# JuanLuisGonzalez/FAL_net

Hardware: AMD Instinct MI355X
Metric: stereo-pairs/sec Stage-1 step @256x512 N=49 (higher is better)
Workload: dtype bf16; 1 GPU; Stage-1 training step (BASELINE configs[1]), batch 8/GPU, 256x512, N=49, seeded weights, seeded VGG19; global_batch=8, parallelism=dp1, launch=eager launches, recorded sequences issued by falnet_replay (C)

## Files before the change

### fal_net_amd/_lib.py

```python
import ctypes as C
import os
import threading

import torch

F32, BF16, F16 = 0, 1, 2
ACT_NONE, ACT_ELU, ACT_RELU = 0, 1, 2
OUT_NHWC, OUT_PLANAR_F32 = 0, 1
CPAD = 32

DETERMINISTIC = os.environ.get("FALNET_DETERMINISTIC") == "1"

def ab(name, default):
    if os.environ.get("FALNET_AB") != "1":
        return default
    return os.environ.get(name, default)


_LIB_PATH = os.environ.get("FALNET_LIB") or os.path.join(os.path.dirname(os.path.abspath(__file__)), "libfalnet_hip.so")


class Src(C.Structure):
    _fields_ = [("ptr", C.c_void_p), ("C", C.c_int32), ("H", C.c_int32), ("W", C.c_int32),
                ("sb", C.c_int64), ("sy", C.c_int64), ("sx", C.c_int64)]


class Conv(C.Structure):
    _fields_ = [("src", Src * 2), ("nsrc", C.c_int32), ("IH", C.c_int32), ("IW", C.c_int32),
                ("weight", C.c_void_p), ("cin_total", C.c_int32), ("ntaps", C.c_int32),
                ("tap_dy", C.c_int32 * 9), ("tap_dx", C.c_int32 * 9), ("tap_w", C.c_int32 * 9),
                ("w_taps", C.c_int32), ("w_rows", C.c_int32), ("isy", C.c_int32), ("isx", C.c_int32),
                ("B", C.c_int32), ("TH", C.c_int32), ("TW", C.c_int32),
                ("osy", C.c_int32), ("osx", C.c_int32), ("ooy", C.c_int32), ("oox", C.c_int32),
                ("out", C.c_void_p), ("OH", C.c_int32), ("OW", C.c_int32), ("Cout", C.c_int32),
                ("out_cstride", C.c_int32), ("out_layout", C.c_int32), ("bias", C.c_void_p),
                ("addend", C.c_void_p), ("act", C.c_int32), ("actout", C.c_void_p),
                ("actout_kind", C.c_int32), ("dtype", C.c_int32), ("ksplit", C.c_int32), ("splitk_ws", C.c_void_p),
                ("splitk_ws_bytes", C.c_int64), ("variant", C.c_int32), ("pool_out", C.c_void_p),
                ("pool_mode", C.c_int32), ("pool_actout_kind", C.c_int32), ("pool_actout", C.c_void_p), ("weight_up2", C.c_void_p),
                ("scratch", C.c_void_p), ("scratch_bytes", C.c_int64), ("pool_code", C.c_void_p)]


class Wgrad(C.Structure):
    _fields_ = [("src", Src * 2), ("nsrc", C.c_int32), ("IH", C.c_int32), ("IW", C.c_int32),
                ("gout", C.c_void_p), ("gC", C.c_int32), ("ntaps", C.c_int32),
                ("tap_dy", C.c_int32 * 9), ("tap_dx", C.c_int32 * 9), ("isy", C.c_int32), ("isx", C.c_int32),
                ("B", C.c_int32), ("TH", C.c_int32), ("TW", C.c_int32), ("cin_total", C.c_int32),
                ("nsplit", C.c_int32), ("partial", C.c_void_p), ("dtype", C.c_int32), ("variant", C.c_int32), ("bias_grad", C.c_void_p),
                ("cout", C.c_int32), ("up2", C.c_int32)]


class ReduceDesc(C.Structure):
    _fields_ = [("partial", C.c_void_p), ("grad", C.c_void_p), ("nsplit", C.c_int32), ("ntaps", C.c_int32),
                ("w_rows", C.c_int32), ("cin_total", C.c_int32), ("cout", C.c_int32), ("cin", C.c_int32),
                ("c0_real", C.c_int32), ("c0_pad", C.c_int32), ("groups", C.c_int32), ("block_begin", C.c_int32)]


class PackDesc(C.Structure):
    _fields_ = [("w", C.c_void_p), ("wf", C.c_void_p), ("wd", C.c_void_p), ("cout", C.c_int32), ("cin", C.c_int32),
                ("taps", C.c_int32), ("c0_real", C.c_int32), ("c0_pad", C.c_int32), ("cin_pad", C.c_int32),
                ("cout_pad", C.c_int32), ("block_begin", C.c_int32), ("no_update", C.c_int32), ("reserved", C.c_int32)]


# ... 407 lines not shown
```

### fal_net_amd/csrc/conv.hip

```cpp
#include <limits.h>
#include <stdlib.h>
#include <type_traits>
#include "common.h"
#include "conv_epilogue.h"

#define CONV_THREADS 256
#define CONV_BM 128
#define ROWB 64
#define ROWP 80

template <typename T> struct KC;
template <> struct KC<float> { static constexpr int value = 16; };
template <> struct KC<bf16_t> { static constexpr int value = 32; };
template <> struct KC<f16_t> { static constexpr int value = 32; };

template <typename T, int MT, int NT, typename RowOff, typename PoolOff = NoPool>
__device__ __forceinline__ void epilogue_nhwc(const falnet_conv_t& p, f32x16 (&acc)[MT][NT], float* stage, int nbase, int lane,
                                              RowOff rowoff, PoolOff pooloff = PoolOff()) {
    constexpr bool POOL = !std::is_same<PoolOff, NoPool>::value;
    constexpr int PITCHF = NT * 32 + 4;
    constexpr int CS = NT * 4;
    constexpr int RPP = 64 / CS;
    constexpr int PASSES = 32 / RPP;
    const int r = lane & 31, h = lane >> 5;
// ... 1466 lines not shown
        }
        flip = fwd ? 0 : (bwd ? 1 : -1);
    }
    dense3x3 = dense3x3 && flip >= 0;
    const int esz = p.dtype == FALNET_F32 ? 4 : 2;
    bool c128 = true;
    for (int s = 0; s < p.nsrc; ++s) c128 = c128 && (p.src[s].C % (128 / esz) == 0);
    int variant = p.variant;
    int forced_bn = 0;
    if (variant == 11 || variant == 12) {
        forced_bn = variant == 11 ? 32 : 64;
        if (p.w_rows % forced_bn != 0 || p.pool_out) {
            falnet_set_error("conv2d: variant %d (gather, %d channels per workgroup) not applicable to this launch", variant, forced_bn);
            return -2;
        }
        variant = 1;
    }
    if (p.pool_code && !(variant == 23 && p.dtype != FALNET_F32 && p.pool_out && p.pool_mode == 0 && !planar && p.OH % 2 == 0 && p.OW % 2 == 0 &&
                         p.Cout % 32 == 0 && p.out_cstride % 32 == 0)) {
        falnet_set_error("conv2d: pool_code (argmax codes of the fused max pool) needs variant 23, a 16-bit type, pool_out with pool_mode 0, an NHWC "
                         "launch with even OH / OW and whole 32-channel groups (variant %d, dtype %d, pool_mode %d)", p.variant, p.dtype, p.pool_mode);
        return -2;
    }
    if (g_disable_patch) variant = 1;
    switch (variant) {
        case 0: case 1: case 2: case 3: case 4: case 5: case 6: case 7: case 8: case 9: case 10:
        case 13: case 15: case 16: case 17: case 18: case 19: case 20: case 21: case 22: case 23: case 24: case 25: case 26: case 27: case 29:
            break;
        default:
            falnet_set_error("conv2d: unknown variant %d", variant);
            return -1;
    }
    if (variant == 19) {
        if (!falnet_conv_deep_applicable(p)) {
            falnet_set_error("conv2d: variant 19 needs a 16-bit nine-tap stride-1/2 launch on maps of at most 128 positions (128 %% (TH TW) == 0), dense NHWC output, "
                             "w_rows %% 64 == 0, ksplit = cin_total / 32 or / 64 (a multiple of 4), scratch for the partial tiles and the split-K workspace");
            return -2;
        }
        c.flip = 0;
        c.swap = 0;
        c.family = ConvFamily::Deep;
        c.bn = 64; c.kcb = p.ksplit * 32 == p.cin_total ? 1 : 2; c.tps = 9; c.adb = 1; c.th = 0; c.nwaves = falnet_conv_deep_mtiles(p);
        return 0;
    }
    if (variant == 15) {
        if (!falnet_conv_s2f_dma_applicable(p)) {
// ... 234 lines not shown
static int ws_symbol(char* buf, int len, const char* t, const falnet_conv_t& p, const ConvChoice& c) {
    const int m16 = (int)(falnet_mfma16_enabled() && p.dtype != FALNET_F32);
    if (c.adb) return snprintf(buf, len, "_Z18conv3x3_ws2_kernelI%sLi%dELi%dELb%dELb%dEEv13falnet_conv_tiii", t, c.bn, c.kcb, m16, (int)(c.kcb == 2 && ws2_whole_lines(p)));
    return snprintf(buf, len, "_Z17conv3x3_ws_kernelI%sLi%dELi%dELb%dEEv13falnet_conv_tiii", t, c.bn, c.kcb, m16);
}

struct ConvFamilyRow {
    ConvFamily family;
    int (*symbol)(char* buf, int len, const char* t, const falnet_conv_t& p, const ConvChoice& c);
    int (*launch)(const falnet_conv_t& p, const ConvChoice& c, hipStream_t st);
};
#define SYMBOL(...) [](char* buf, int len, const char* t, const falnet_conv_t& p, const ConvChoice& c) { return snprintf(buf, len, __VA_ARGS__); }
#define LAUNCH(...) [](const falnet_conv_t& p, const ConvChoice& c, hipStream_t st) { return __VA_ARGS__; }
static const ConvFamilyRow conv_families[] = {
    {ConvFamily::Gather, SYMBOL("_Z17conv_igemm_kernelI%sLi%dELb%dEEv13falnet_conv_t", t, c.bn, c.swap), launch_gather},
    {ConvFamily::Patch, SYMBOL("_Z20conv3x3_patch_kernelI%sLi%dELi%dELi%dELb%dELi%dELi%dEEv13falnet_conv_tiii", t, c.bn, c.kcb, c.tps, c.adb, c.th, c.nwaves), launch_patch},
    {ConvFamily::WeightStationary, ws_symbol, launch_ws},
    {ConvFamily::Dma, SYMBOL("_Z18conv3x3_dma_kernelI%sLi%dELi%dEEv13falnet_conv_tiiii", t, c.th, c.nwaves), LAUNCH(falnet_conv_dma_launch(p, c.flip, st, c.th, c.max_wgs, c.count))},
    {ConvFamily::S2fDma, SYMBOL("_Z22conv3x3_s2f_dma_kernelI%sLi%dEEv13falnet_conv_tiii", t, c.bn), LAUNCH(falnet_conv_s2f_dma_launch(p, st, c.max_wgs, c.count))},
    {ConvFamily::Up2Dma, SYMBOL("_Z22conv3x3_up2_dma_kernelI%sEv13falnet_conv_tiiiii", t), LAUNCH(falnet_conv_up2_dma_launch(p, st, c.max_wgs, c.count))},
    {ConvFamily::Deep, SYMBOL("_Z19conv3x3_deep_kernelI%sLi%dELi%dEEv13falnet_conv_t18falnet_deep_geom_t", t, c.kcb, c.nwaves), LAUNCH(falnet_conv_deep_launch(p, st, c.count))},
    {ConvFamily::Dma2, SYMBOL("_Z19conv3x3_dma2_kernelI%sLb%dELi%dEEv13falnet_conv_tiiiii", t, p.pool_out ? 1 : 0, c.nwaves), LAUNCH(falnet_conv_dma2_launch(p, c.flip, st, c.th, c.max_wgs, c.count))},
    {ConvFamily::Dma16, [](char* buf, int len, const char* t, const falnet_conv_t& p, const ConvChoice& c) {
         if (p.pool_out && p.pool_code) return snprintf(buf, len, "_Z20conv3x3_dma16_kernelI9PoolCodesI%sELb1ELi16ELi8ELb0EEv13falnet_conv_tiiii", t);
         return snprintf(buf, len, "_Z20conv3x3_dma16_kernelI%sLb%dELi%dELi%dELb%dEEv13falnet_conv_tiiii", t, p.pool_out ? 1 : 0, c.th, c.nwaves, p.out_layout == FALNET_OUT_PLANAR_F32 ? 1 : 0);
     },
     LAUNCH(falnet_conv_dma16_launch(p, c.flip, st, c.th, c.max_wgs, c.count))},
    {ConvFamily::Up2d, SYMBOL("_Z25conv2x2_up2d_dma16_kernelI%sEv13falnet_conv_tiii", t), LAUNCH(falnet_conv_up2d_launch(p, st, c.max_wgs, c.count))},
    {ConvFamily::Wave32, SYMBOL("_Z21conv3x3_wave32_kernelI%sEv13falnet_conv_tiiii", t), LAUNCH(falnet_conv_wave32_launch(p, c.flip, st, c.count))},
    {ConvFamily::Wave64p, SYMBOL("_Z22conv3x3_wave64p_kernelI%sEv13falnet_conv_tiiii", t), LAUNCH(falnet_conv_wave64p_launch(p, c.flip, st, c.count))},
};
#undef SYMBOL
#undef LAUNCH

static const ConvFamilyRow* conv_family_row(ConvFamily f) {
    for (const ConvFamilyRow& r : conv_families)
        if (r.family == f) return &r;
    falnet_set_error("conv2d: kernel family %d has no table row", (int)f);
    return nullptr;
}

extern "C" int falnet_conv2d_kernel_name(const falnet_conv_t* pp, char* buf, int len) {
    FALNET_CHECK_ARG(pp && buf && len > 0, "conv2d_kernel_name: bad argument");
    ConvChoice c;
    if (int r = choose_conv_kernel(*pp, c)) return r;
    const ConvFamilyRow* row = conv_family_row(c.family);
// ... 155 lines not shown
```

### fal_net_amd/csrc/conv_dma.hip

```cpp
#include <stdlib.h>
#include "conv_epilogue.h"

#ifndef FALNET_DMA_ROW_REUSE
#define FALNET_DMA_ROW_REUSE 1
#endif
#ifndef FALNET_DMA_EPI_AHEAD
#define FALNET_DMA_EPI_AHEAD -1
#endif
#ifndef FALNET_DMA16_EPI_AHEAD
#define FALNET_DMA16_EPI_AHEAD 0
#endif

#define CD_ZERO_BYTES 32768
__device__ uint4 g_cd_zero[CD_ZERO_BYTES / 16] = {};

typedef __attribute__((address_space(3))) void* cd_lptr_t;

__device__ __forceinline__ void cd_glds16(const void* gsrc, unsigned lds_dst) {
    unsigned keep;
    asm volatile("s_mov_b32 %0, m0\n\ts_mov_b32 m0, %2\n\ts_nop 0\n\tglobal_load_lds_dwordx4 %1, off\n\ts_mov_b32 m0, %0"
                 : "=&s"(keep)
                 : "v"(gsrc), "s"(lds_dst)
                 : "memory");
}
// ... 535 lines not shown
    FALNET_COUNT_ONLY(count, gx * ny);
    static const int skew_pct = [] { const char* e = falnet_ab_env("FALNET_DMA2_SKEW"); return e ? atoi(e) : 0; }();
    int cin = 0;
    for (int s = 0; s < p.nsrc; ++s) cin += p.src[s].C;
    const int skew = (th == 16 && gx * ny > 256) ? (int)((int64_t)skew_pct * (cin / 16) * 5200 / 100 / 64) : 0;
#define DMA2_K(T, PL, NW) hipLaunchKernelGGL(HIP_KERNEL_NAME(conv3x3_dma2_kernel<T, PL, NW>), grid, dim3(NW * 64), 0, st, p, tiles_x, tiles_y, flip, ntiles, skew)
#define DMA2_L(T)                                              \
    do {                                                       \
        if (th == 32) {                                        \
            if (p.pool_out) DMA2_K(T, true, 8);                \
            else DMA2_K(T, false, 8);                          \
        } else {                                               \
            if (p.pool_out) DMA2_K(T, true, 4);                \
            else DMA2_K(T, false, 4);                          \
        }                                                      \
    } while (0)
    FALNET_DISPATCH_16(p.dtype, DMA2_L);
#undef DMA2_L
#undef DMA2_K
    FALNET_RETURN_LAUNCH();
}

template <typename T> struct PoolCodes {};
template <typename TT> struct Dma16Operand { typedef TT type; static constexpr bool codes = false; };
template <typename T> struct Dma16Operand<PoolCodes<T>> { typedef T type; static constexpr bool codes = true; };
template <typename TT, bool POOL, int TH, int NWAVES, bool PLANAR>
__global__ __launch_bounds__(NWAVES * 64, NWAVES == 8 ? 2 : 1) void conv3x3_dma16_kernel(const falnet_conv_t p, int tiles_x, int tiles_y, int flip, int ntiles) {
    typedef typename Dma16Operand<TT>::type T;
    constexpr bool CODES = Dma16Operand<TT>::codes;
    constexpr int MT = TH / NWAVES, BN = 64, NT = BN / 32;
    static_assert(sizeof(T) == 2 && (MT == 1 || MT == 2) && (MT == 2 || !POOL), "16-bit operands; one or two rows per wave; the fused pool needs row pairs");
    constexpr int KCV = 32;
    constexpr int NPIX = (TH + 2) * CD_PW;
    constexpr int A_PIECES = (NPIX + 15) / 16, B_PIECES = 9 * BN / 16, NPIECES = A_PIECES + B_PIECES;
    constexpr int A_BYTES = A_PIECES * 1024, BUF = NPIECES * 1024;
    constexpr int ROWB = CD_PW * 64;
    __shared__ __attribute__((aligned(1024))) char lds[2 * BUF];
    __shared__ __attribute__((aligned(16))) float lds_bias[BN];
    const int tid = threadIdx.x, lane = tid & 63;
    const int wave = __builtin_amdgcn_readfirstlane(tid >> 6);
    const unsigned lds_base = (unsigned)(unsigned long)(cd_lptr_t)lds;
    const int r = lane & 31, h = lane >> 5;
    const int lp = lane & 15, lg = lane >> 4;
    const int n0 = blockIdx.y * BN;
    const char* const zero_page = reinterpret_cast<const char*>(g_cd_zero);
    stage_bias_lds(p, n0, BN, lds_bias);

    const int nsrc = p.nsrc, IH = p.IH, IW = p.IW;
    const int C0 = p.src[0].C, C1 = nsrc > 1 ? p.src[1].C : 0;
    const int nchunks = (C0 + C1) / KCV;
    int my_tiles = 0;
    for (int t = blockIdx.x; t < ntiles; t += gridDim.x) ++my_tiles;
// ... 33 lines not shown
        t.tx += step_.tx;
        if (t.tx >= tiles_x) { t.tx -= tiles_x; ++t.ty; }
        t.ty += step_.ty;
        if (t.ty >= tiles_y) { t.ty -= tiles_y; ++t.b; }
        t.b += step_.b;
    };
    int pr_[KP], pc_[KP], a_lc[2][KP];
#pragma unroll
    for (int k = 0; k < KP; ++k) {
        const int pix = 16 * (wave + NWAVES * k) + l4;
        const int pr = pix / CD_PW, pc = pix - pr * CD_PW;
        pr_[k] = pix < NPIX ? pr : -(1 << 20);
        pc_[k] = pc;
#pragma unroll
        for (int s2 = 0; s2 < 2; ++s2) {
            const falnet_src_t& S = s2 == 0 ? p.src[0] : p.src[(nsrc > 1) ? 1 : 0];
            const int hs = S.H != IH ? 1 : 0, ws = S.W != IW ? 1 : 0;
            a_lc[s2][k] = ((pr - 1) >> hs) * (int)S.sy + ((pc - 1) >> ws) * (int)S.sx + (segpos ^ (((pc >> 2) & 1) << 1)) * 8;
        }
    }
    int a_off[KP];
    unsigned a_ok = 0;
    const T* a_base = sptr[0];
    auto tile_offsets = [&](const TPos& t, int s2) {
        const falnet_src_t& S = s2 == 0 ? p.src[0] : p.src[1];
        const int hs = S.H != IH ? 1 : 0, ws = S.W != IW ? 1 : 0;
        const int ty0 = t.ty * TH, tx0 = t.tx * 32;
        a_base = sptr[s2] + ((int64_t)t.b * S.sb + (int64_t)((ty0 >> hs) * (int)S.sy + (tx0 >> ws) * (int)S.sx));
        a_ok = 0;
#pragma unroll
        for (int k = 0; k < KP; ++k) {
            const int vy = ty0 - 1 + pr_[k], vx = tx0 - 1 + pc_[k];
            a_ok |= (vy >= 0 && vy < IH && vx >= 0 && vx < IW) ? 1u << k : 0u;
            a_off[k] = a_lc[s2][k];
        }
    };
    struct Cur { int tile, c, s, c0, kofs; TPos t; };
    auto advance = [&](Cur& q) {
        if (++q.c == nchunks) {
            q.c = 0; q.s = 0; q.c0 = 0; q.kofs = 0;
            q.tile += gridDim.x;
            pos_next(q.t);
            if (q.tile < ntiles) tile_offsets(q.t, 0);
            return;
        }
        q.c0 += KCV;
        q.kofs += KCV;
        if (q.s == 0 && q.c0 >= C0) {
            q.s = 1;
            q.c0 = 0;
            tile_offsets(q.t, 1);
        }
    };
    auto issue_piece = [&](const Cur& q, int buf, int i) {
        const unsigned dst0 = lds_base + buf * BUF;
        if (i < KP) {
            const int id = wave + NWAVES * i;
            const T* src = ((a_ok >> i) & 1) ? a_base + q.c0 + a_off[i] : zero_t;
            if (id < A_PIECES) cd_glds16(src, dst0 + id * 1024);
        } else {
            const int wid = wave + NWAVES * (i - KP);
            if (wid < B_PIECES) cd_glds16(wptr + q.kofs + w_off[i - KP], dst0 + A_BYTES + wid * 1024);
        }
    };

    int a_lane[3][2];
#pragma unroll
    for (int dx = 0; dx < 3; ++dx)
#pragma unroll
        for (int pt = 0; pt < 2; ++pt) {
            const int col = dx + 16 * pt + lp;
            a_lane[dx][pt] = ((wave * MT) * CD_PW + col) * 64 + ((lg ^ (((col >> 2) & 1) << 1)) << 4);
        }
    const int wrow = m16_row_channel(lp);
    const int b_lane = A_BYTES + wrow * 64 + ((lg ^ (((wrow >> 2) & 1) << 1)) << 4);

    Acc16 acc[MT][NT];
#pragma unroll
    for (int mt = 0; mt < MT; ++mt)
#pragma unroll
        for (int nt = 0; nt < NT; ++nt) acc[mt][nt].zero();
    Cur qi = {(int)blockIdx.x, 0, 0, 0, 0, pos_of((int)blockIdx.x)};
// ... 11 lines not shown
#define CD16_STAMP()                                                                                 \
    do {                                                                                             \
        __builtin_amdgcn_sched_barrier(0);                                                           \
        unsigned long long t_;                                                                       \
        asm volatile("s_memtime %0\n\ts_waitcnt lgkmcnt(0)" : "=s"(t_)::"memory");                  \
        __builtin_amdgcn_sched_barrier(0);                                                           \
        if (stamp_out && blockIdx.x == 0 && blockIdx.y == 0 && lane == 0 && stamp_i < 256) stamp_out[wave * 256 + stamp_i] = t_; \
        ++stamp_i;                                                                                   \
    } while (0)
#else
#define CD16_STAMP() do {} while (0)
#endif
#if defined(FALNET_CD_STAMPS) && FALNET_CD_STAMPS == 2
#define CD16_A() do {} while (0)
#define CD16_B() CD16_STAMP()
#else
#define CD16_A() CD16_STAMP()
#define CD16_B() do {} while (0)
#endif
    for (int it = 0; it < total; ++it) {
        CD16_STAMP();
        asm volatile("s_waitcnt vmcnt(0) lgkmcnt(0)" ::: "memory");
        CD16_A();
        __builtin_amdgcn_s_barrier();
        CD16_STAMP();
        CD16_A();
        const bool more = it + 1 < total;
        int bo = (it & 1) * BUF;
        asm volatile("" : "+s"(bo));
        const char* const Bf = lds;
        int aa[3][2];
#pragma unroll
        for (int dx = 0; dx < 3; ++dx)
#pragma unroll
            for (int pt = 0; pt < 2; ++pt) aa[dx][pt] = a_lane[dx][pt] + bo;
        const int bb = b_lane + bo;
        s16x8_t fa[3][MT + 2][2], fb[2][NT][2];
        auto a_read = [&](int dx, int rs, int pt) { return *reinterpret_cast<const s16x8_t*>(Bf + aa[dx][pt] + rs * ROWB); };
        auto b_read = [&](int st, int set) {
            const int t = (st % 3) * 3 + st / 3;
#pragma unroll
            for (int nt = 0; nt < NT; ++nt)
#pragma unroll
                for (int ct = 0; ct < 2; ++ct) fb[set][nt][ct] = *reinterpret_cast<const s16x8_t*>(Bf + bb + (t * BN + nt * 32 + ct * 16) * 64);
        };
        static_assert(KP + KW <= 18, "two DMA issue slots per step");
// ... 73 lines not shown
            CD16_B();
        }
        CD16_STAMP();
    }
#undef CD16_STAMP
#undef CD16_A
#undef CD16_B
}

int falnet_conv_dma16_launch(const falnet_conv_t& p, int flip, hipStream_t st, int th, int max_wgs, int* count) {
    const int tiles_x = (p.OW + 31) / 32, tiles_y = (p.OH + th - 1) / th;
    const int ntiles = p.B * tiles_x * tiles_y;
    const int ny = (p.Cout + 63) / 64;
    const int gx = falnet_persistent_gx(256, ny, ntiles, max_wgs);
    const dim3 grid((unsigned)gx, (unsigned)ny);
    FALNET_COUNT_ONLY(count, gx * ny);
    const bool planar = p.out_layout == FALNET_OUT_PLANAR_F32;
#define DMA16_K(T, PL, TH_, NW, PN) hipLaunchKernelGGL(HIP_KERNEL_NAME(conv3x3_dma16_kernel<T, PL, TH_, NW, PN>), grid, dim3(NW * 64), 0, st, p, tiles_x, tiles_y, flip, ntiles)
#define DMA16_L(T)                                        \
    do {                                                  \
        if (th == 4) DMA16_K(T, false, 4, 4, false);      \
        else if (th == 8) DMA16_K(T, false, 8, 8, false); \
        else if (planar) DMA16_K(T, false, 16, 8, true);  \
        else if (p.pool_out && p.pool_code) DMA16_K(PoolCodes<T>, true, 16, 8, false); \
        else if (p.pool_out) DMA16_K(T, true, 16, 8, false); \
        else DMA16_K(T, false, 16, 8, false);             \
    } while (0)
    FALNET_DISPATCH_16(p.dtype, DMA16_L);
#undef DMA16_L
#undef DMA16_K
    FALNET_RETURN_LAUNCH();
}

template <typename T>
__global__ __launch_bounds__(512, 2) void conv2x2_up2d_dma16_kernel(const falnet_conv_t p, int tiles_x, int tiles_y, int ntiles) {
    constexpr int TH = 16, NWAVES = 8, MT = 2, BN = 64, NT = 2, KCV = 32;
    constexpr int NPIX = (TH + 1) * CD_PW;
    constexpr int A_PIECES = (NPIX + 15) / 16, B_PIECES = 4 * BN / 16, NPIECES = A_PIECES + B_PIECES;
    constexpr int A_BYTES = A_PIECES * 1024, BUF = NPIECES * 1024;
    constexpr int ROWB = CD_PW * 64;
    __shared__ __attribute__((aligned(1024))) char lds[2 * BUF];
    __shared__ __attribute__((aligned(16))) float lds_bias[BN];
    const int tid = threadIdx.x, lane = tid & 63;
    const int wave = __builtin_amdgcn_readfirstlane(tid >> 6);
    const unsigned lds_base = (unsigned)(unsigned long)(cd_lptr_t)lds;
    const int r = lane & 31;
// ... 1175 lines not shown
```

### fal_net_amd/loss_functions.py

```python
import os
import weakref

import torch
import torch.nn as nn
import torch.nn.functional as F

from . import _lib as L
from . import ops, synthetic
from .ops import PackedConv

_MEAN = (0.411, 0.432, 0.45)
_SLICES = ((0, 2), (5, 7), (10, 12, 14, 16))


_GOUT_OF = {}
_MAX_HELD_PLANS = 4


def _forget_gouts(keys):
    for k in keys:
        _GOUT_OF.pop(k, None)


def _release_plan(plan, gen):
    if plan.gen == gen:
        plan.busy = False


class _VggPlan:

    def __init__(self, owner, B, H, W, dtype, device, need_grad=True, pool_codes=None, pool_variant=None, max_wgs=None):
        assert not (max_wgs and need_grad), "a workgroup budget is for the gradient-free label pass"
        self.max_wgs = max_wgs or 0
        self.B, self.H, self.W, self.dtype, self.device = B, H, W, dtype, device
        self.busy, self.need_grad, self.gen = False, need_grad, 0
        if pool_codes is None:
            pool_codes = L.ab("FALNET_POOL_CODES", "1") == "1"
        self.pool_maps, self.pool_codes = [], []
        code = L.dtype_code(dtype)
        self.fwd, self.bwd = [], []
        _conv = lambda *a, **kw: ops.conv_call(*a, ws_owner=("vgg", id(self)), max_wgs=self.max_wgs, **kw)
        pcs = owner._packed
        x_in = torch.empty(B, 3, H, W, dtype=torch.float32, device=device)
        x0 = x_in
        self.x_in, self.keep = x_in, []
        cur, h, w = x0, H, W
        self.outs, acts = [], []
        for convs in _SLICES:
            for idx in convs:
                pc = pcs[idx]
                last = idx == convs[-1]
                pooled = torch.empty(B, h // 2, w // 2, pc.cout, dtype=dtype, device=device) if last else None
                codes = None
                kw = dict(bias=pc.bias, act=L.ACT_RELU, name=f"vgg conv{idx}", flops=2 * B * h * w * pc.cout * pc.cin * 9)
# ... 28 lines not shown
                acts.append((pc, cur, y, h, w))
                cur = y
            acts.append(("pool", cur, pooled, h, w, codes))
            self.pool_maps.append(cur)
            self.pool_codes.append(codes)
            self.outs.append(pooled)
            cur, h, w = pooled, h // 2, w // 2
        if self.max_wgs and os.environ.get("FALNET_AUTOTUNE_LOG") == "1":
            import sys
            for c in self.fwd:
                if getattr(c, "max_wgs", 0):
                    full, cut = (L.lib().falnet_conv2d_workgroups(c.ref, m) for m in (0, c.max_wgs))
                    print(f"[label budget {self.max_wgs}] {c.name}: {full} -> {cut} workgroups", file=sys.stderr)
        self.run_fwd = ops.ReplayList(self.fwd, eager_head=1)
        self.run_bwd = None
        if not need_grad:
            return
        self.gouts = [torch.empty_like(o) for o in self.outs]
        for o, g in zip(self.outs, self.gouts):
            _GOUT_OF[o.data_ptr()] = [g, False]
        weakref.finalize(self, _forget_gouts, [o.data_ptr() for o in self.outs])
        g_next = None
        slice_i = len(self.outs) - 1
        for entry in reversed(acts):
            if entry[0] == "pool":
                _, x, pooled, h, w, codes = entry
                gy = self.gouts[slice_i] if g_next is None else g_next
                ch = pooled.shape[3]
                gx = torch.empty(B, h, w, ch, dtype=dtype, device=device)
                if codes is not None:
                    self.bwd.append(ops.simple_call("falnet_maxpool2_bwd_codes", L.ptr(codes), L.ptr(gy), L.ptr(gx), B, h, w, ch, code))
                    self.keep.append(codes)
                else:
                    self.bwd.append(ops.simple_call("falnet_maxpool2_bwd", L.ptr(x), L.ptr(pooled), L.ptr(gy), L.ptr(gx), B, h, w, ch, code))
                g_next, slice_i = gx, slice_i - 1
                self.keep.append(gx)
            else:
                pc, x, y, h, w = entry
                if x is x0:
                    self.g_in = torch.empty(B, 3, H, W, dtype=torch.float32, device=device)
                    self.bwd.append(_conv(dtype, [ops.nhwc_src(g_next)], h, w, pc.wd, pc.cout_pad, ops.dgrad_taps_s1(3), 9,
                                          ops.pad_c(3), 1, B, h, w, self.g_in, h, w, 3, 0, out_layout=L.OUT_PLANAR_F32, name="vgg dgrad0",
                                          flops=2 * B * h * w * pc.cout * pc.cin * 9))
                else:
                    from_pool = any(x is o for o in self.outs)
                    gin = torch.empty_like(x)
                    own = next((g for o, g in zip(self.outs, self.gouts) if x is o), None)
                    self.bwd.append(_conv(dtype, [ops.nhwc_src(g_next)], h, w, pc.wd, pc.cout_pad, ops.dgrad_taps_s1(3), 9,
                                                  pc.cin_pad, 1, B, h, w, gin, h, w, pc.cin_pad, pc.cin_pad, addend=own,
                                                  actout=None if from_pool else x,
                                                  actout_kind=L.ACT_NONE if from_pool else L.ACT_RELU, name="vgg dgrad",
                                                  flops=2 * B * h * w * pc.cout * pc.cin * 9))
                    self.keep.append(gin)
                    g_next = gin
        self.run_bwd = ops.ReplayList(self.bwd)


class _VggFunction(torch.autograd.Function):
    @staticmethod
    def forward(ctx, owner, plan, x):
        plan.c3_call.set_input(x)
        plan.run_fwd()
        ctx.plan, ctx.owner, ctx.gen = plan, owner, plan.gen
        weakref.finalize(ctx, _release_plan, plan, plan.gen)
        return tuple(o.permute(0, 3, 1, 2) for o in plan.outs)

    @staticmethod
    def backward(ctx, *gouts):
        plan = ctx.plan
        if plan.gen != ctx.gen:
            raise RuntimeError(f"this VGG call's plan was recycled: more than {_MAX_HELD_PLANS} grad-enabled vgg() calls of one shape "
                               "were alive without a backward")
        for buf, g in zip(plan.gouts, gouts):
            if g is None:
                buf.zero_()
            elif g.data_ptr() != buf.data_ptr():
                buf.copy_(g.permute(0, 2, 3, 1))
        plan.run_bwd()
# ... 22 lines not shown
            p.requires_grad = requires_grad
        self.compute_dtype = compute_dtype
        self._plans, self._packed, self._packed_key = {}, None, None

    def _prepare(self, device, dtype):
        key = (device, dtype)
        if self._packed_key != key:
            if next(self.parameters()).device != device:
                self.to(device)
            self._packed = {}
            for i, conv in self.features.items():
                pc = PackedConv(f"vgg{i}", conv.weight, conv.bias, [conv.weight.shape[1]], 1)
                pc.alloc(dtype, device)
                pc.pack_call()()
                self._packed[int(i)] = pc
            self._packed_key, self._plans = key, {}

    def _plan(self, B, H, W, dtype, device, hold, max_wgs=0):
        pool = self._plans.setdefault((B, H, W, hold, max_wgs) if max_wgs else (B, H, W, hold), [])
        p = next((q for q in pool if not q.busy), None)
        if p is None and hold and len(pool) >= _MAX_HELD_PLANS:
            p = min(pool, key=lambda q: q.gen)
        if p is None:
            p = _VggPlan(self, B, H, W, dtype, device, need_grad=hold, max_wgs=max_wgs)
            pool.append(p)
        self._gen = getattr(self, "_gen", 0) + 1
        p.busy, p.gen = hold, self._gen
        if hold:
            for o in p.outs:
                _GOUT_OF[o.data_ptr()][1] = False
        return p

    def forward(self, x, full=False, borrow=False, max_wgs=0):
        if full:
            raise NotImplementedError("slice4 (relu4_4) is never used on the FAL_net hot path (loss_functions.py:40-42)")
        if not x.is_cuda:
            raise RuntimeError("fal_net_amd Vgg19_pc runs on an MI355X only (no CPU fallback)")
        dtype = self.compute_dtype or _default_dtype()
        self._prepare(x.device, dtype)
        B, C, H, W = x.shape
        assert C == 3 and H % 8 == 0 and W % 8 == 0, "VGG19 slices need a 3-channel input with H, W divisible by 8"
        need_grad = torch.is_grad_enabled() and x.requires_grad
        plan = self._plan(B, H, W, dtype, x.device, hold=need_grad, max_wgs=0 if need_grad else int(max_wgs or 0))
        xs = x.float().contiguous() if need_grad else x.detach().float().contiguous()
        if need_grad:
            return _VggFunction.apply(self, plan, xs)
        with torch.no_grad():
# ... 253 lines not shown
```

### fal_net_amd/ops.py

```python
import ctypes as C
import os
import sys

import torch

from . import _lib as L

CPAD = L.CPAD
H16 = (torch.bfloat16, torch.float16)
TYPE_SYM = {torch.bfloat16: "DF16b", torch.float16: "DF16_", torch.float32: "f"}

TIMER = None
AUTOTUNE = os.environ.get("FALNET_AUTOTUNE", "1") != "0"
DETERMINISTIC = L.DETERMINISTIC
UP2W = L.ab("FALNET_UP2W", "0") == "1"
UP2Q = frozenset(k for k in L.ab("FALNET_UP2Q", "deconv1,deconv2,deconv3,deconv4").split(",") if k)
UP2D = L.ab("FALNET_UP2D", "1") == "1"


_PKG_CACHE = os.path.join(os.path.dirname(os.path.abspath(__file__)), "autotune_cache.json")
_CACHE_PATH = os.environ.get("FALNET_AUTOTUNE_CACHE", _PKG_CACHE)
_CACHE_WRITABLE = ("FALNET_AUTOTUNE_CACHE" in os.environ and _CACHE_PATH != "0") or os.environ.get("FALNET_AUTOTUNE_CACHE_WRITE") == "1"
_GATES = {"FALNET_NO_DMA": "0", "FALNET_WS2": "1", "FALNET_S2F_DMA": "1", "FALNET_S2D_DMA": "1", "FALNET_S2_SPLITK": "1",
          "FALNET_GATHER_NARROW": "0", "FALNET_S2_MULTI": None, "FALNET_SMALL_TILE_DMA": "1", "FALNET_UP2": "1", "FALNET_DEEP": "1", "FALNET_TILE8": "1"}
# ... 50 lines not shown
    if not _CACHE_DIRTY or _CACHE_PATH == "0" or not _CACHE_WRITABLE:
        return
    try:
        import json
        tmp = _CACHE_PATH + f".{os.getpid()}.tmp"
        with open(tmp, "w") as f:
            json.dump({"_meta": cache_meta(), **dict(sorted(_cache().items()))}, f, indent=0)
        os.replace(tmp, _CACHE_PATH)
        _CACHE_DIRTY = False
    except OSError:
        pass


import atexit
atexit.register(cache_flush)


def conv_signature(d):
    srcs = ";".join(f"{d.src[i].C},{d.src[i].H},{d.src[i].W},{int(d.src[i].sy == 0)}" for i in range(d.nsrc))
    taps = ",".join(f"{d.tap_dy[t]}:{d.tap_dx[t]}:{d.tap_w[t]}" for t in range(d.ntaps))
    flags = f"{int(bool(d.bias))}{int(bool(d.addend))}{d.act}{int(bool(d.actout))}{d.actout_kind}{int(bool(d.pool_out))}{d.pool_mode}{int(bool(d.pool_actout))}{int(bool(d.out))}"
    return (f"conv|t{d.dtype}|{srcs}|{d.IH}x{d.IW}|k{d.cin_total}|{taps}|w{d.w_taps}x{d.w_rows}|s{d.isy}|B{d.B}|{d.TH}x{d.TW}|"
            f"o{d.osy},{d.ooy},{d.oox}|{d.OH}x{d.OW}|c{d.Cout},{d.out_cstride},{d.out_layout}|f{flags}|ws{int(d.splitk_ws_bytes > 0)}"
            + ("|up2" if d.weight_up2 else ""))


_PROBE_SKIP = [x for x in L.ab("FALNET_PROBE_SKIP", "").split(",") if x]


def _timed(tag, flops, nbytes, launch, name=""):
    if _PROBE_SKIP and any(x in name for x in _PROBE_SKIP):
        launch = lambda *a: None
    def call(*a):
        t = TIMER
        if t is None:
            launch(*a)
        else:
            t.run(tag, flops, nbytes, lambda: launch(*a), name)
    call.tag, call.flops, call.nbytes, call.name = tag, flops, nbytes, name
    return call


def pad_c(c):
    return (c + CPAD - 1) // CPAD * CPAD


def nhwc_src(t, C_used=None):
# ... 179 lines not shown
    taps = []
    for kh in range(3):
        if (py + 1 - kh) % 2:
            continue
        for kw in range(3):
            if (px + 1 - kw) % 2:
                continue
            taps.append(((py + 1 - kh) // 2, (px + 1 - kw) // 2, kh * 3 + kw))
    return taps


def _fill_taps(d, taps):
    d.ntaps = len(taps)
    for i, (dy, dx, w) in enumerate(taps):
        d.tap_dy[i], d.tap_dx[i] = dy, dx
        if hasattr(d, "tap_w"):
            d.tap_w[i] = w


def conv_call(dtype, srcs, IH, IW, weight, cin_total, taps, w_taps, w_rows, stride_in, B, TH, TW, out, OH, OW,
              Cout, out_cstride, out_layout=L.OUT_NHWC, out_step=(1, 1, 0, 0), bias=None, addend=None,
              act=L.ACT_NONE, actout=None, actout_kind=L.ACT_NONE, weight_offset_elems=0, name="conv", flops=0,
              autotune=True, ws_owner=None, pool_out=None, pool_mode=0, pool_actout=None, pool_actout_kind=L.ACT_NONE, weight_up2=None,
              variant=None, pool_code=None, max_wgs=None):
    lib = L.lib()
    if max_wgs is not None and max_wgs < 0:
        raise ValueError(f"max_wgs = {max_wgs}: a workgroup budget is None / 0 (the full grid) or positive")
    d = L.Conv()
    d.nsrc = len(srcs)
    for i, s in enumerate(srcs):
        d.src[i] = s
    d.IH, d.IW = IH, IW
    d.weight = weight.data_ptr() + weight_offset_elems * weight.element_size()
    d.cin_total, d.w_taps, d.w_rows = cin_total, w_taps, w_rows
    _fill_taps(d, taps)
    d.isy = d.isx = stride_in
    d.B, d.TH, d.TW = B, TH, TW
    d.osy, d.osx, d.ooy, d.oox = out_step
    d.out, d.OH, d.OW, d.Cout, d.out_cstride, d.out_layout = (0 if out is None else out.data_ptr()), OH, OW, Cout, out_cstride, out_layout
    d.pool_out = 0 if pool_out is None else pool_out.data_ptr()
    d.pool_mode, d.pool_actout_kind = pool_mode, pool_actout_kind
    d.pool_actout = 0 if pool_actout is None else pool_actout.data_ptr()
    d.weight_up2 = 0 if weight_up2 is None else weight_up2.data_ptr()
    d.pool_code = 0 if pool_code is None else pool_code.data_ptr()
    dev_t = out if out is not None else pool_out
    d.bias = 0 if bias is None else bias.data_ptr()
    d.addend = 0 if addend is None else addend.data_ptr()
    d.act = act
    d.actout = 0 if actout is None else actout.data_ptr()
    d.actout_kind = actout_kind
    d.dtype = L.dtype_code(dtype)
    d.variant = 0
    d.ksplit = 1
    ws = _splitk_workspace(dev_t.device, ws_owner) if dev_t.is_cuda and out_layout == L.OUT_NHWC and pool_out is None else None
    d.splitk_ws = 0 if ws is None else ws.data_ptr()
    d.splitk_ws_bytes = 0 if ws is None else ws.numel() * 4
    scratch = None
    if ws is not None and dtype in H16 and TH * TW <= 128 and len(taps) == 9:
        scratch = _deep_scratch(dev_t.device, ws_owner)
        d.scratch, d.scratch_bytes = scratch.data_ptr(), scratch.numel() * 4
    ref = C.byref(d)
    keep = (d, srcs, weight, out, bias, addend, actout, ws, pool_out, pool_actout, weight_up2, scratch, pool_code)
    if variant is not None:
        d.variant = variant
        if lib.falnet_conv2d_kernel_name(ref, C.create_string_buffer(160), 160) != 0:
            raise ValueError(f"falnet_conv2d variant {variant} does not apply to this launch: {lib.falnet_last_error().decode(errors='replace')}")
    elif AUTOTUNE and autotune and dev_t.is_cuda:
        key = conv_signature(d)
        hit = cache_get(key)
        if hit is not None:
            d.variant, d.ksplit = int(hit[0]), int(hit[1])
            if DETERMINISTIC and d.ksplit > 1 and d.variant != 19:
                d.variant, d.ksplit = 1, 1
            if lib.falnet_conv2d_kernel_name(ref, C.create_string_buffer(160), 160) != 0:
                hit = None
        if hit is None and DETERMINISTIC:
            d.variant, d.ksplit = 0, 1
        elif hit is None:
            d.variant, d.ksplit = _autotune_conv(lib, d, ref, B * TH * TW, w_rows, Cout)
            cache_put(key, [int(d.variant), int(d.ksplit)])
    if pool_out is not None and lib.falnet_conv2d_kernel_name(ref, C.create_string_buffer(160), 160) != 0:
        raise ValueError("no fused-pool kernel applies to this launch")

    if max_wgs:
        def launch(_keep=keep):
# ... 516 lines not shown
```

### include/falnet_hip.h

```cpp
#ifndef FALNET_HIP_H
#define FALNET_HIP_H

#include <stdint.h>

#ifdef __cplusplus
extern "C" {
#endif

enum { FALNET_F32 = 0, FALNET_BF16 = 1, FALNET_F16 = 2 };
enum { FALNET_ACT_NONE = 0, FALNET_ACT_ELU = 1, FALNET_ACT_RELU = 2 };
enum { FALNET_OUT_NHWC = 0, FALNET_OUT_PLANAR_F32 = 1 };

int falnet_version(void);
const char* falnet_last_error(void);
int falnet_channel_pad(int dtype);
int falnet_set_device(int device);
int falnet_set_deterministic(int on);
int falnet_get_deterministic(void);

typedef struct {
    const void* ptr;
    int32_t C;
    int32_t H, W;
    int64_t sb, sy, sx;
// ... 14 lines not shown
    int32_t osy, osx, ooy, oox;
    void* out;
    int32_t OH, OW;
    int32_t Cout;
    int32_t out_cstride;
    int32_t out_layout;
    const float* bias;
    const void* addend;
    int32_t act;
    const void* actout;
    int32_t actout_kind;
    int32_t dtype;
    int32_t ksplit;
    float* splitk_ws;
    int64_t splitk_ws_bytes;
    int32_t variant;
    void* pool_out;
    int32_t pool_mode;
    int32_t pool_actout_kind;
    const void* pool_actout;
    const void* weight_up2;
    void* scratch;
    int64_t scratch_bytes;
    void* pool_code;
} falnet_conv_t;
int falnet_conv2d(const falnet_conv_t* p, void* stream);
int falnet_conv2d_wgs(const falnet_conv_t* p, int max_workgroups, void* stream);
int falnet_conv2d_workgroups(const falnet_conv_t* p, int max_workgroups);
int falnet_conv3x3_c3(const float* x_nchw, const float* w_oihw, const float* bias, void* out, int B, int H, int W, int Cout,
                      int act, int dtype, void* stream);
int falnet_conv2d_multi(const falnet_conv_t* descs, int n, void* stream);
int falnet_conv2d_multi_wgs(const falnet_conv_t* descs, int n, int max_workgroups, void* stream);
int falnet_conv2d_kernel_name(const falnet_conv_t* p, char* buf, int len);

typedef struct {
    falnet_src_t src[2];
    int32_t nsrc;
    int32_t IH, IW;
    const void* gout;
    int32_t gC;
    int32_t ntaps;
    int32_t tap_dy[9], tap_dx[9];
    int32_t isy, isx;
    int32_t B, TH, TW;
    int32_t cin_total;
    int32_t nsplit;
// ... 276 lines not shown
```

Before: 1693 stereo-pairs/s.

## Fuse max-pool backward into the following VGG dgrad conv via argmax codes

Adds a src_code path to the dma16 conv kernel. The kernel reads the half-resolution pooled gradient directly, loads the per-channel argmax codes alongside each A tile, and masks in LDS every element that did not win the pool. This removes the separate maxpool2_bwd_codes expand kernel and the full-resolution gradient buffer it writes and then reads back. The loss plan benchmarks fused against split per layer and caches the choice. The cost is extra code loads, an LDS masking pass and an additional wait before the barrier in the main loop.

```diff
diff --git a/fal_net_amd/_lib.py b/fal_net_amd/_lib.py
--- a/fal_net_amd/_lib.py
+++ b/fal_net_amd/_lib.py
@@ -38,7 +38,7 @@
                 ("actout_kind", C.c_int32), ("dtype", C.c_int32), ("ksplit", C.c_int32), ("splitk_ws", C.c_void_p),
                 ("splitk_ws_bytes", C.c_int64), ("variant", C.c_int32), ("pool_out", C.c_void_p),
                 ("pool_mode", C.c_int32), ("pool_actout_kind", C.c_int32), ("pool_actout", C.c_void_p), ("weight_up2", C.c_void_p),
-                ("scratch", C.c_void_p), ("scratch_bytes", C.c_int64), ("pool_code", C.c_void_p)]
+                ("scratch", C.c_void_p), ("scratch_bytes", C.c_int64), ("src_code", C.c_void_p), ("pool_code", C.c_void_p)]
 
 
 class Wgrad(C.Structure):
diff --git a/fal_net_amd/csrc/conv.hip b/fal_net_amd/csrc/conv.hip
--- a/fal_net_amd/csrc/conv.hip
+++ b/fal_net_amd/csrc/conv.hip
@@ -1512,6 +1512,16 @@
                          "launch with even OH / OW and whole 32-channel groups (variant %d, dtype %d, pool_mode %d)", p.variant, p.dtype, p.pool_mode);
         return -2;
     }
+    if (p.src_code) {
+        const falnet_src_t& S = p.src[0];
+        if (!(variant == 23 && p.dtype != FALNET_F32 && p.nsrc == 1 && !planar && !p.pool_out && S.C > 0 && S.C % 32 == 0 && 2 * S.H == p.IH && 2 * S.W == p.IW &&
+              S.sx == S.C && S.sy == (int64_t)S.W * S.C && S.sb == (int64_t)S.H * S.W * S.C && reinterpret_cast<uintptr_t>(p.src_code) % 4 == 0)) {
+            falnet_set_error("conv2d: src_code (argmax codes of the max pool whose output gradient is the source) needs variant 23, a 16-bit type, ONE dense NHWC "
+                             "source at exactly half the launch size with whole 32-channel groups, 4-byte aligned codes, an NHWC launch without a fused pool "
+                             "(variant %d, dtype %d, nsrc %d, C %d, source %d x %d for %d x %d)", p.variant, p.dtype, p.nsrc, S.C, S.H, S.W, p.IH, p.IW);
+            return -2;
+        }
+    }
     if (g_disable_patch) variant = 1;
     switch (variant) {
         case 0: case 1: case 2: case 3: case 4: case 5: case 6: case 7: case 8: case 9: case 10:
@@ -1792,6 +1802,7 @@
     {ConvFamily::Deep, SYMBOL("_Z19conv3x3_deep_kernelI%sLi%dELi%dEEv13falnet_conv_t18falnet_deep_geom_t", t, c.kcb, c.nwaves), LAUNCH(falnet_conv_deep_launch(p, st, c.count))},
     {ConvFamily::Dma2, SYMBOL("_Z19conv3x3_dma2_kernelI%sLb%dELi%dEEv13falnet_conv_tiiiii", t, p.pool_out ? 1 : 0, c.nwaves), LAUNCH(falnet_conv_dma2_launch(p, c.flip, st, c.th, c.max_wgs, c.count))},
     {ConvFamily::Dma16, [](char* buf, int len, const char* t, const falnet_conv_t& p, const ConvChoice& c) {
+         if (p.src_code) return snprintf(buf, len, "_Z20conv3x3_dma16_kernelI9PoolDgradI%sELb0ELi16ELi8ELb0EEv13falnet_conv_tiiii", t);
          if (p.pool_out && p.pool_code) return snprintf(buf, len, "_Z20conv3x3_dma16_kernelI9PoolCodesI%sELb1ELi16ELi8ELb0EEv13falnet_conv_tiiii", t);
          return snprintf(buf, len, "_Z20conv3x3_dma16_kernelI%sLb%dELi%dELi%dELb%dEEv13falnet_conv_tiiii", t, p.pool_out ? 1 : 0, c.th, c.nwaves, p.out_layout == FALNET_OUT_PLANAR_F32 ? 1 : 0);
      },
diff --git a/fal_net_amd/csrc/conv_dma.hip b/fal_net_amd/csrc/conv_dma.hip
--- a/fal_net_amd/csrc/conv_dma.hip
+++ b/fal_net_amd/csrc/conv_dma.hip
@@ -581,12 +581,24 @@
 }
 
 template <typename T> struct PoolCodes {};
-template <typename TT> struct Dma16Operand { typedef TT type; static constexpr bool codes = false; };
-template <typename T> struct Dma16Operand<PoolCodes<T>> { typedef T type; static constexpr bool codes = true; };
+template <typename T> struct PoolDgrad {};
+template <typename TT> struct Dma16Operand { typedef TT type; static constexpr bool codes = false, src_codes = false; };
+template <typename T> struct Dma16Operand<PoolCodes<T>> { typedef T type; static constexpr bool codes = true, src_codes = false; };
+template <typename T> struct Dma16Operand<PoolDgrad<T>> { typedef T type; static constexpr bool codes = false, src_codes = true; };
+__device__ __forceinline__ uint4 cd_keep_winners(uint4 v, unsigned cw, int bit) {
+    const unsigned t = cw >> bit;
+    const unsigned tl = t & 0x01010101u, th = (t >> 4) & 0x01010101u;
+    const unsigned ml = (tl << 8) - tl, mh = (th << 8) - th;
+    v.x &= __builtin_amdgcn_perm(mh, ml, 0x04040000u);
+    v.y &= __builtin_amdgcn_perm(mh, ml, 0x05050101u);
+    v.z &= __builtin_amdgcn_perm(mh, ml, 0x06060202u);
+    v.w &= __builtin_amdgcn_perm(mh, ml, 0x07070303u);
+    return v;
+}
 template <typename TT, bool POOL, int TH, int NWAVES, bool PLANAR>
 __global__ __launch_bounds__(NWAVES * 64, NWAVES == 8 ? 2 : 1) void conv3x3_dma16_kernel(const falnet_conv_t p, int tiles_x, int tiles_y, int flip, int ntiles) {
     typedef typename Dma16Operand<TT>::type T;
-    constexpr bool CODES = Dma16Operand<TT>::codes;
+    constexpr bool CODES = Dma16Operand<TT>::codes, SRCC = Dma16Operand<TT>::src_codes;
     constexpr int MT = TH / NWAVES, BN = 64, NT = BN / 32;
     static_assert(sizeof(T) == 2 && (MT == 1 || MT == 2) && (MT == 2 || !POOL), "16-bit operands; one or two rows per wave; the fused pool needs row pairs");
     constexpr int KCV = 32;
@@ -666,11 +678,15 @@
     int a_off[KP];
     unsigned a_ok = 0;
     const T* a_base = sptr[0];
+    const unsigned char* const code0 = reinterpret_cast<const unsigned char*>(p.src_code);
+    const unsigned char* c_base = code0;
+    unsigned cw[KP];
     auto tile_offsets = [&](const TPos& t, int s2) {
         const falnet_src_t& S = s2 == 0 ? p.src[0] : p.src[1];
         const int hs = S.H != IH ? 1 : 0, ws = S.W != IW ? 1 : 0;
         const int ty0 = t.ty * TH, tx0 = t.tx * 32;
         a_base = sptr[s2] + ((int64_t)t.b * S.sb + (int64_t)((ty0 >> hs) * (int)S.sy + (tx0 >> ws) * (int)S.sx));
+        if constexpr (SRCC) c_base = code0 + ((a_base - sptr[0]) >> 1);
         a_ok = 0;
 #pragma unroll
         for (int k = 0; k < KP; ++k) {
@@ -700,8 +716,12 @@
         const unsigned dst0 = lds_base + buf * BUF;
         if (i < KP) {
             const int id = wave + NWAVES * i;
-            const T* src = ((a_ok >> i) & 1) ? a_base + q.c0 + a_off[i] : zero_t;
-            if (id < A_PIECES) cd_glds16(src, dst0 + id * 1024);
+            const bool ok = (a_ok >> i) & 1;
+            const T* src = ok ? a_base + q.c0 + a_off[i] : zero_t;
+            if (id < A_PIECES) {
+                cd_glds16(src, dst0 + id * 1024);
+                if constexpr (SRCC) cw[i] = *reinterpret_cast<const unsigned*>(ok ? c_base + ((q.c0 + a_off[i]) >> 1) : code0);
+            }
         } else {
             const int wid = wave + NWAVES * (i - KP);
             if (wid < B_PIECES) cd_glds16(wptr + q.kofs + w_off[i - KP], dst0 + A_BYTES + wid * 1024);
@@ -759,6 +779,16 @@
         CD16_STAMP();
         asm volatile("s_waitcnt vmcnt(0) lgkmcnt(0)" ::: "memory");
         CD16_A();
+        if constexpr (SRCC) {
+#pragma unroll
+            for (int k = 0; k < KP; ++k) {
+                if (wave + NWAVES * k < A_PIECES) {
+                    uint4* const q = reinterpret_cast<uint4*>(lds + (it & 1) * BUF + (wave + NWAVES * k) * 1024 + lane * 16);
+                    *q = cd_keep_winners(*q, cw[k], (((pr_[k] + 1) & 1) << 1) | ((pc_[k] + 1) & 1));
+                }
+            }
+            asm volatile("s_waitcnt lgkmcnt(0)" ::: "memory");
+        }
         __builtin_amdgcn_s_barrier();
         CD16_STAMP();
         CD16_A();
@@ -878,6 +908,7 @@
         if (th == 4) DMA16_K(T, false, 4, 4, false);      \
         else if (th == 8) DMA16_K(T, false, 8, 8, false); \
         else if (planar) DMA16_K(T, false, 16, 8, true);  \
+        else if (p.src_code) DMA16_K(PoolDgrad<T>, false, 16, 8, false); \
         else if (p.pool_out && p.pool_code) DMA16_K(PoolCodes<T>, true, 16, 8, false); \
         else if (p.pool_out) DMA16_K(T, true, 16, 8, false); \
         else DMA16_K(T, false, 16, 8, false);             \
diff --git a/fal_net_amd/loss_functions.py b/fal_net_amd/loss_functions.py
--- a/fal_net_amd/loss_functions.py
+++ b/fal_net_amd/loss_functions.py
@@ -29,7 +29,7 @@
 
 class _VggPlan:
 
-    def __init__(self, owner, B, H, W, dtype, device, need_grad=True, pool_codes=None, pool_variant=None, max_wgs=None):
+    def __init__(self, owner, B, H, W, dtype, device, need_grad=True, pool_codes=None, pool_variant=None, max_wgs=None, pool_dgrad=False):
         assert not (max_wgs and need_grad), "a workgroup budget is for the gradient-free label pass"
         self.max_wgs = max_wgs or 0
         self.B, self.H, self.W, self.dtype, self.device = B, H, W, dtype, device
@@ -104,17 +104,22 @@
         weakref.finalize(self, _forget_gouts, [o.data_ptr() for o in self.outs])
         g_next = None
         slice_i = len(self.outs) - 1
+        if pool_dgrad is None:
+            pool_dgrad = L.ab("FALNET_POOL_DGRAD", "1") == "1"
+        pending = None
+        self.pool_dgrad = []
         for entry in reversed(acts):
             if entry[0] == "pool":
                 _, x, pooled, h, w, codes = entry
                 gy = self.gouts[slice_i] if g_next is None else g_next
                 ch = pooled.shape[3]
+                if codes is not None:
+                    pending = (gy, codes, ch)
+                    self.keep.append(codes)
+                    g_next, slice_i = gy, slice_i - 1
+                    continue
                 gx = torch.empty(B, h, w, ch, dtype=dtype, device=device)
-                if codes is not None:
-                    self.bwd.append(ops.simple_call("falnet_maxpool2_bwd_codes", L.ptr(codes), L.ptr(gy), L.ptr(gx), B, h, w, ch, code))
-                    self.keep.append(codes)
-                else:
-                    self.bwd.append(ops.simple_call("falnet_maxpool2_bwd", L.ptr(x), L.ptr(pooled), L.ptr(gy), L.ptr(gx), B, h, w, ch, code))
+                self.bwd.append(ops.simple_call("falnet_maxpool2_bwd", L.ptr(x), L.ptr(pooled), L.ptr(gy), L.ptr(gx), B, h, w, ch, code))
                 g_next, slice_i = gx, slice_i - 1
                 self.keep.append(gx)
             else:
@@ -128,14 +133,52 @@
                     from_pool = any(x is o for o in self.outs)
                     gin = torch.empty_like(x)
                     own = next((g for o, g in zip(self.outs, self.gouts) if x is o), None)
-                    self.bwd.append(_conv(dtype, [ops.nhwc_src(g_next)], h, w, pc.wd, pc.cout_pad, ops.dgrad_taps_s1(3), 9,
-                                                  pc.cin_pad, 1, B, h, w, gin, h, w, pc.cin_pad, pc.cin_pad, addend=own,
-                                                  actout=None if from_pool else x,
-                                                  actout_kind=L.ACT_NONE if from_pool else L.ACT_RELU, name="vgg dgrad",
-                                                  flops=2 * B * h * w * pc.cout * pc.cin * 9))
+                    def dgrad(g, name="vgg dgrad", **extra):
+                        return _conv(dtype, [ops.nhwc_src(g)], h, w, pc.wd, pc.cout_pad, ops.dgrad_taps_s1(3), 9,
+                                     pc.cin_pad, 1, B, h, w, gin, h, w, pc.cin_pad, pc.cin_pad, addend=own,
+                                     actout=None if from_pool else x,
+                                     actout_kind=L.ACT_NONE if from_pool else L.ACT_RELU, name=name,
+                                     flops=2 * B * h * w * pc.cout * pc.cin * 9, **extra)
+                    if pending is not None:
+                        (gy, codes, ch), pending = pending, None
+                        self.bwd += self._pool_dgrad(dgrad, gy, codes, ch, h, w, code, pool_dgrad)
+                    else:
+                        self.bwd.append(dgrad(g_next))
                     self.keep.append(gin)
                     g_next = gin
         self.run_bwd = ops.ReplayList(self.bwd)
+
+    def _pool_dgrad(self, dgrad, gy, codes, ch, h, w, code, enabled):
+        B, dtype, device = self.B, self.dtype, self.device
+
+        def split(variant=None):
+            gx = torch.empty(B, h, w, ch, dtype=dtype, device=device)
+            self.keep.append(gx)
+            expand = ops.simple_call("falnet_maxpool2_bwd_codes", L.ptr(codes), L.ptr(gy), L.ptr(gx), B, h, w, ch, code)
+            try:
+                return [expand, dgrad(gx, variant=variant)]
+            except ValueError:
+                return [expand, dgrad(gx)]
+        if not enabled:
+            self.pool_dgrad.append(False)
+            return split(23 if ops.DETERMINISTIC else None)
+        try:
+            fused = [dgrad(gy, name="vgg dgrad+pool", src_code=codes, variant=23)]
+        except ValueError:
+            self.pool_dgrad.append(False)
+            return split()
+        key = "pooldgrad|" + ops.conv_signature(fused[0].desc)
+        hit = ops.cache_get(key)
+        if hit is None and not ops.DETERMINISTIC:
+            cands = [fused, split()]
+            runs = [lambda seq=seq: [c() for c in seq] for seq in cands]
+            pick = cands[runs.index(ops.best_of(*runs, key=key))]
+            if pick is fused:
+                self.keep.pop()
+        else:
+            pick = fused if not hit else split()
+        self.pool_dgrad.append(pick is fused)
+        return pick
 
 
 class _VggFunction(torch.autograd.Function):
@@ -204,7 +247,7 @@
         if p is None and hold and len(pool) >= _MAX_HELD_PLANS:
             p = min(pool, key=lambda q: q.gen)
         if p is None:
-            p = _VggPlan(self, B, H, W, dtype, device, need_grad=hold, max_wgs=max_wgs)
+            p = _VggPlan(self, B, H, W, dtype, device, need_grad=hold, max_wgs=max_wgs, pool_dgrad=None)
             pool.append(p)
         self._gen = getattr(self, "_gen", 0) + 1
         p.busy, p.gen = hold, self._gen
diff --git a/fal_net_amd/ops.py b/fal_net_amd/ops.py
--- a/fal_net_amd/ops.py
+++ b/fal_net_amd/ops.py
@@ -96,7 +96,7 @@
     flags = f"{int(bool(d.bias))}{int(bool(d.addend))}{d.act}{int(bool(d.actout))}{d.actout_kind}{int(bool(d.pool_out))}{d.pool_mode}{int(bool(d.pool_actout))}{int(bool(d.out))}"
     return (f"conv|t{d.dtype}|{srcs}|{d.IH}x{d.IW}|k{d.cin_total}|{taps}|w{d.w_taps}x{d.w_rows}|s{d.isy}|B{d.B}|{d.TH}x{d.TW}|"
             f"o{d.osy},{d.ooy},{d.oox}|{d.OH}x{d.OW}|c{d.Cout},{d.out_cstride},{d.out_layout}|f{flags}|ws{int(d.splitk_ws_bytes > 0)}"
-            + ("|up2" if d.weight_up2 else ""))
+            + ("|up2" if d.weight_up2 else "") + ("|srccode" if d.src_code else ""))
 
 
 _PROBE_SKIP = [x for x in L.ab("FALNET_PROBE_SKIP", "").split(",") if x]
@@ -322,7 +322,7 @@
               Cout, out_cstride, out_layout=L.OUT_NHWC, out_step=(1, 1, 0, 0), bias=None, addend=None,
               act=L.ACT_NONE, actout=None, actout_kind=L.ACT_NONE, weight_offset_elems=0, name="conv", flops=0,
               autotune=True, ws_owner=None, pool_out=None, pool_mode=0, pool_actout=None, pool_actout_kind=L.ACT_NONE, weight_up2=None,
-              variant=None, pool_code=None, max_wgs=None):
+              variant=None, pool_code=None, max_wgs=None, src_code=None):
     lib = L.lib()
     if max_wgs is not None and max_wgs < 0:
         raise ValueError(f"max_wgs = {max_wgs}: a workgroup budget is None / 0 (the full grid) or positive")
@@ -343,6 +343,7 @@
     d.pool_actout = 0 if pool_actout is None else pool_actout.data_ptr()
     d.weight_up2 = 0 if weight_up2 is None else weight_up2.data_ptr()
     d.pool_code = 0 if pool_code is None else pool_code.data_ptr()
+    d.src_code = 0 if src_code is None else src_code.data_ptr()
     dev_t = out if out is not None else pool_out
     d.bias = 0 if bias is None else bias.data_ptr()
     d.addend = 0 if addend is None else addend.data_ptr()
@@ -360,7 +361,7 @@
         scratch = _deep_scratch(dev_t.device, ws_owner)
         d.scratch, d.scratch_bytes = scratch.data_ptr(), scratch.numel() * 4
     ref = C.byref(d)
-    keep = (d, srcs, weight, out, bias, addend, actout, ws, pool_out, pool_actout, weight_up2, scratch, pool_code)
+    keep = (d, srcs, weight, out, bias, addend, actout, ws, pool_out, pool_actout, weight_up2, scratch, pool_code, src_code)
     if variant is not None:
         d.variant = variant
         if lib.falnet_conv2d_kernel_name(ref, C.create_string_buffer(160), 160) != 0:
diff --git a/include/falnet_hip.h b/include/falnet_hip.h
--- a/include/falnet_hip.h
+++ b/include/falnet_hip.h
@@ -60,6 +60,7 @@
     const void* weight_up2;
     void* scratch;
     int64_t scratch_bytes;
+    const void* src_code;
     void* pool_code;
 } falnet_conv_t;
 int falnet_conv2d(const falnet_conv_t* p, void* stream);
```

Result: no change. 1706 stereo-pairs/s, median of 6 (+0.8%).
